# Sovik-Ghosh/SFM

Measured on AMD Instinct MI355X. Metric: BA LM-iterations/sec + descriptor-pairs/sec, 200 cams / 100k pts, 1->8 MI355X, higher is better.
Workload: dtype f64; 1 GPU; BA: 200 cams / 100000 pts / 1000000 obs, cam block 10 (reference 10-parameter block + regulariser), aligned residual order, Huber, SciPy-TRF control flow, fixed schedule; parallelism=points sharded over 1 rank(s), cameras replicated, RCCL all-reduce of [S|r], comm=single rank, seed=1004

## Files before the change

sfm_amd/csrc/ba_model.hip:

```cpp
#include "ba_internal.h"
#include "ba_device.h"

template <int D>
__global__ void k_campre(const double* __restrict__ cams, int C, double fx0, double fy0, double cx0,
                         double cy0, double* __restrict__ out) {
  int c = blockIdx.x * blockDim.x + threadIdx.x;
  if (c >= C) return;
  const double* p = cams + (size_t)c * D;
  const double th2 = p[0] * p[0] + p[1] * p[1] + p[2] * p[2];
  double a, b, a1, b1;
  if (th2 < 1e-4) {
    double z = th2;
    a = 1.0 - z / 6.0 + z * z / 120.0;
    b = 0.5 - z / 24.0 + z * z / 720.0;
    a1 = -1.0 / 3.0 + z / 30.0 - z * z / 840.0;
    b1 = -1.0 / 12.0 + z / 180.0 - z * z / 6720.0;
  } else {
    double t = sqrt(th2), s, co;
    sincos(t, &s, &co);
    a = s / t;
    b = (1.0 - co) / th2;
    a1 = (t * co - s) / (th2 * t);
    b1 = (t * s - 2.0 * (1.0 - co)) / (th2 * th2);
  }
  double* o = out + (size_t)c * CAMPRE;
#pragma unroll
  for (int i = 0; i < 6; ++i) o[i] = p[i];
  if (D == 10) { o[6] = p[6]; o[7] = p[7]; o[8] = p[8]; o[9] = p[9]; }
  else { o[6] = fx0; o[7] = fy0; o[8] = cx0; o[9] = cy0; }
  o[10] = a; o[11] = b; o[12] = a1; o[13] = b1; o[14] = th2; o[15] = 0.0;
}

__device__ __forceinline__ void cam_project(const double* __restrict__ cp, double X0, double X1, double X2,
                                            double& Y0, double& Y1, double& Y2) {
  const double r0 = cp[0], r1 = cp[1], r2 = cp[2], a = cp[10], b = cp[11];
  const double c0 = r1 * X2 - r2 * X1, c1 = r2 * X0 - r0 * X2, c2 = r0 * X1 - r1 * X0;
  const double e0 = r1 * c2 - r2 * c1, e1 = r2 * c0 - r0 * c2, e2 = r0 * c1 - r1 * c0;
  Y0 = X0 + a * c0 + b * e0 + cp[3];
  Y1 = X1 + a * c1 + b * e1 + cp[4];
  Y2 = X2 + a * c2 + b * e2 + cp[5];
}

template <int D, typename T>
__global__ __launch_bounds__(256) void k_lin_obs(int64_t N, const int* __restrict__ cam_idx,
                                                 const int* __restrict__ pt_idx,
                                                 const double* __restrict__ uv,
                                                 const double* __restrict__ pts,
                                                 const double* __restrict__ campre,
                                                 T* __restrict__ recA, T* __restrict__ recB,
                                                 double* __restrict__ part) {
  constexpr int WA = 2 * D, LDA = WA + 1, WB = 8, LDB = WB + 1;
  __shared__ double s_rec[256 * LDA];
  __shared__ double s_red[4];
  const int tid = threadIdx.x;
  const int64_t k0 = (int64_t)blockIdx.x * 256;
  const int64_t k = k0 + tid;
  double cost = 0.0;
  double jb[8];
#pragma unroll
  for (int q = 0; q < 8; ++q) jb[q] = 0.0;
  if (k < N) {
    const int c = cam_idx[k], j = pt_idx[k];
    const double* cp = campre + (size_t)c * CAMPRE;
// ... 41 lines not shown
    const double R10 = a * r2 + b * r1 * r0, R11 = 1.0 + b * (r1 * r1 - th2), R12 = -a * r0 + b * r1 * r2;
    const double R20 = -a * r1 + b * r2 * r0, R21 = a * r0 + b * r2 * r1, R22 = 1.0 + b * (r2 * r2 - th2);
    jb[0] = p00 * R00 + p02 * R20; jb[1] = p00 * R01 + p02 * R21; jb[2] = p00 * R02 + p02 * R22;
    jb[3] = p11 * R10 + p12 * R20; jb[4] = p11 * R11 + p12 * R21; jb[5] = p11 * R12 + p12 * R22;
    jb[6] = ft0; jb[7] = ft1;
  }
  double tot = block_sum256(cost, s_red);
  if (tid == 0) part[blockIdx.x] = tot;
  const int nvalid = (int)((N - k0) < 256 ? (N - k0) : 256);
  {
    T* outp = recA + (size_t)k0 * WA;
    for (int i = tid; i < nvalid * WA; i += 256) {
      const int t = i / WA, q = i - t * WA;
      outp[i] = (T)s_rec[t * LDA + q];
    }
  }
  __syncthreads();
  {
    double* my = &s_rec[tid * LDB];
#pragma unroll
    for (int q = 0; q < 8; ++q) my[q] = jb[q];
  }
  __syncthreads();
  {
    T* outp = recB + (size_t)k0 * WB;
    for (int i = tid; i < nvalid * WB; i += 256) {
      const int t = i >> 3, q = i & 7;
      outp[i] = (T)s_rec[t * LDB + q];
    }
  }
}

template <typename T>
__global__ __launch_bounds__(256) void k_point_blocks(int P, const int* __restrict__ pt_ptr,
                                                      const T* __restrict__ recB,
                                                      double* __restrict__ Cp, double* __restrict__ gp,
                                                      double* __restrict__ part) {
  __shared__ double s_red[4];
  const int j = blockIdx.x * 256 + threadIdx.x;
  double g2 = 0.0, gm = 0.0, cm = 0.0;
  if (j < P) {
    double c0 = 0, c1 = 0, c2 = 0, c3 = 0, c4 = 0, c5 = 0, g0 = 0, g1 = 0, g2v = 0;
    for (int k = pt_ptr[j]; k < pt_ptr[j + 1]; ++k) {
      const T* r = recB + (size_t)k * 8;
      const double a0 = r[0], a1 = r[1], a2 = r[2], b0 = r[3], b1 = r[4], b2 = r[5], f0 = r[6], f1 = r[7];
      c0 += a0 * a0 + b0 * b0; c1 += a0 * a1 + b0 * b1; c2 += a0 * a2 + b0 * b2;
      c3 += a1 * a1 + b1 * b1; c4 += a1 * a2 + b1 * b2; c5 += a2 * a2 + b2 * b2;
      g0 += a0 * f0 + b0 * f1; g1 += a1 * f0 + b1 * f1; g2v += a2 * f0 + b2 * f1;
    }
    double* co = Cp + (size_t)j * 6;
    co[0] = c0; co[1] = c1; co[2] = c2; co[3] = c3; co[4] = c4; co[5] = c5;
    gp[(size_t)j * 3] = g0; gp[(size_t)j * 3 + 1] = g1; gp[(size_t)j * 3 + 2] = g2v;
    g2 = g0 * g0 + g1 * g1 + g2v * g2v;
    gm = fmax(fabs(g0), fmax(fabs(g1), fabs(g2v)));
    cm = fmax(c0, fmax(c3, c5));
  }
  double t2 = block_sum256(g2, s_red);
  double tm = block_max256(gm, s_red);
  double tc = block_max256(cm, s_red);
  if (threadIdx.x == 0) { part[blockIdx.x * 4] = t2; part[blockIdx.x * 4 + 1] = tm; part[blockIdx.x * 4 + 2] = tc; }
}

template <int D, typename T>
__global__ __launch_bounds__(256) void k_cam_blocks_chunks(const int* __restrict__ cch_beg, const int* __restrict__ cch_end,
                                                           const int* __restrict__ cam_obs,
                                                           const T* __restrict__ recA,
                                                           const T* __restrict__ recB, double* __restrict__ part) {
  constexpr int W = 2 * D + 2, LDW = W + 1, NE = D * D + D;
  __shared__ double s[256 * LDW];
  __shared__ double s_tile[4][16 * 17];
  const int ch = blockIdx.x, tid = threadIdx.x, lane = tid & 63, w = tid >> 6;
  const int beg = cch_beg[ch], cnt = cch_end[ch] - beg;
  {
    typedef T pair_t __attribute__((ext_vector_type(2)));
    const int slot = tid >> 4, l16 = tid & 15;
    const bool live = l16 <= D;
    int kk[16];
#pragma unroll
    for (int it = 0; it < 16; ++it) {
      const int o = it * 16 + slot;
      kk[it] = (live && o < cnt) ? cam_obs[beg + o] : -1;
    }
    pair_t v[16];
#pragma unroll
    for (int it = 0; it < 16; ++it) {
      v[it] = (pair_t)(T)0;
      if (kk[it] >= 0)
        v[it] = l16 < D ? *(const pair_t*)(recA + (size_t)kk[it] * (2 * D) + 2 * l16) : *(const pair_t*)(recB + (size_t)kk[it] * 8 + 6);
    }
#pragma unroll
    for (int it = 0; it < 16; ++it) {
      const int o = it * 16 + slot;
      if (kk[it] >= 0) { s[o * LDW + 2 * l16] = (double)v[it].x; s[o * LDW + 2 * l16 + 1] = (double)v[it].y; }
    }
  }
  __syncthreads();
  const int col = lane & 15, kq = lane >> 4;
  const int rrow = kq & 1;
  const int q = col < D ? rrow * D + col : 2 * D + rrow;
  const bool live = col <= D;
  const int per = (cnt + 3) / 4;
  const int wu = __builtin_amdgcn_readfirstlane(w);
  const int o0 = wu * per, o1 = (o0 + per) < cnt ? (o0 + per) : cnt;
  v4d acc = {0.0, 0.0, 0.0, 0.0};
  for (int o = o0; o < o1; o += 8) {
    double v[4];
#pragma unroll
    for (int u = 0; u < 4; ++u) {
      const int oo = o + 2 * u + (kq >> 1);
      v[u] = (live && oo < o1) ? s[oo * LDW + q] : 0.0;
    }
#pragma unroll
    for (int u = 0; u < 4; ++u) {
      if (o + 2 * u >= o1) break;
      acc = __builtin_amdgcn_mfma_f64_16x16x4f64(v[u], v[u], acc, 0, 0, 0);
    }
  }
#pragma unroll
  for (int i = 0; i < 4; ++i) s_tile[w][(kq + 4 * i) * 17 + col] = acc[i];
  __syncthreads();
  if (tid < NE) {
    const int a = tid < D * D ? tid / D : tid - D * D;
    const int b = tid < D * D ? tid - a * D : D;
    part[(size_t)ch * NE + tid] = ((s_tile[0][a * 17 + b] + s_tile[1][a * 17 + b]) + s_tile[2][a * 17 + b]) + s_tile[3][a * 17 + b];
  }
}
template <int D>
__global__ void k_cam_blocks_final(int C, const int* __restrict__ cch_ptr, const double* __restrict__ part,
                                   double* __restrict__ B, double* __restrict__ gc) {
  constexpr int NE = D * D + D;
  const int i = blockIdx.x * blockDim.x + threadIdx.x;
  if (i >= C * NE) return;
  const int c = i / NE, e = i - c * NE;
  double t = 0.0;
  for (int ch = cch_ptr[c]; ch < cch_ptr[c + 1]; ++ch) t += part[(size_t)ch * NE + e];
  if (e < D * D) B[(size_t)c * D * D + e] = t;
  else gc[(size_t)c * D + (e - D * D)] = t;
}

__global__ void k_cam_reg(int C, const double* __restrict__ cams, double fx0, double cx0, double cy0,
                          double width, double height, double w, double* __restrict__ B,
                          double* __restrict__ gc, double* __restrict__ cost_reg,
                          double* __restrict__ regrec) {
  const int c = blockIdx.x * blockDim.x + threadIdx.x;
  if (c >= C) return;
  const double* p = cams + (size_t)c * 10;
  const double fx = p[6], fy = p[7], cx = p[8], cy = p[9];
  double f[4] = {(fx - fx0) / fx0 * w, (fy - fx) / fx * w, (cx - cx0) / width * w, (cy - cy0) / height * w};
  double J[16];
#pragma unroll
  for (int i = 0; i < 16; ++i) J[i] = 0.0;
  J[0] = w / fx0;
  J[4] = -w * fy / (fx * fx); J[5] = w / fx;
  J[10] = w / width;
  J[15] = w / height;
  double cost = 0.0, ft[4];
#pragma unroll
  for (int r = 0; r < 4; ++r) {
    double sc;
    cost += huber_row(f[r], sc, ft[r]);
#pragma unroll
    for (int q = 0; q < 4; ++q) J[r * 4 + q] *= sc;
  }
  cost_reg[c] = 0.5 * cost;
  double* Bc = B + (size_t)c * 100;
#pragma unroll
  for (int i = 0; i < 4; ++i) {
    double g = 0.0;
#pragma unroll
    for (int r = 0; r < 4; ++r) g += J[r * 4 + i] * ft[r];
    gc[(size_t)c * 10 + 6 + i] += g;
#pragma unroll
    for (int q = 0; q < 4; ++q) {
      double hsum = 0.0;
#pragma unroll
      for (int r = 0; r < 4; ++r) hsum += J[r * 4 + i] * J[r * 4 + q];
      Bc[(6 + i) * 10 + 6 + q] += hsum;
    }
  }
  double* rr = regrec + (size_t)c * 20;
#pragma unroll
  for (int i = 0; i < 16; ++i) rr[i] = J[i];
#pragma unroll
  for (int r = 0; r < 4; ++r) rr[16 + r] = ft[r];
}

__global__ __launch_bounds__(256) void k_lin_finalize(int n, int D, const double* __restrict__ gc,
                                                      const double* __restrict__ B,
                                                      const double* __restrict__ part_obs, int nblk_obs,
                                                      const double* __restrict__ part_pt, int nblk_pt,
                                                      const double* __restrict__ cost_reg, int n_reg,
                                                      double* __restrict__ red_lin, double* __restrict__ gmax) {
  __shared__ double s_red[4];
  const int tid = threadIdx.x;
  #pragma unroll 8
  for (int i = tid; i < n; i += 256) {
    red_lin[i] = gc[i];
    const int cam = i / D, a = i - cam * D;
    red_lin[n + 2 + i] = B[(size_t)cam * D * D + a * D + a];
  }
  double c = 0.0, g2 = 0.0, gm = 0.0, cm = 0.0;
  #pragma unroll 8
  for (int i = tid; i < nblk_obs; i += 256) c += part_obs[i];
  #pragma unroll 8
  for (int i = tid; i < n_reg; i += 256) c += cost_reg[i];
  #pragma unroll 8
  for (int i = tid; i < nblk_pt; i += 256) { g2 += part_pt[4 * i]; gm = fmax(gm, part_pt[4 * i + 1]); cm = fmax(cm, part_pt[4 * i + 2]); }
  double ct = block_sum256(c, s_red);
  double g2t = block_sum256(g2, s_red);
  double gmt = block_max256(gm, s_red);
  double cmt = block_max256(cm, s_red);
  if (tid == 0) { red_lin[n] = ct; red_lin[n + 1] = g2t; gmax[0] = gmt; gmax[1] = cmt; }
}

__global__ __launch_bounds__(256) void k_finish_linearize(int n, const double* __restrict__ red_lin,
                                                          const double* __restrict__ gmax,
                                                          double* __restrict__ sc, double* __restrict__ hsc, double seq) {
  __shared__ double s_red[4];
  double g2 = 0.0, gm = 0.0, hm = 0.0;
  #pragma unroll 8
  for (int i = threadIdx.x; i < n; i += 256) {
    double v = red_lin[i]; g2 += v * v; gm = fmax(gm, fabs(v));
    hm = fmax(hm, red_lin[n + 2 + i]);
  }
  double g2t = block_sum256(g2, s_red);
  double gmt = block_max256(gm, s_red);
  double hmt = block_max256(hm, s_red);
  if (threadIdx.x == 0) {
    sc[SFM_SC_COST] = hsc[SFM_SC_COST] = red_lin[n];
    sc[SFM_SC_GNORM2] = hsc[SFM_SC_GNORM2] = g2t + red_lin[n + 1];
    sc[SFM_SC_GINF] = hsc[SFM_SC_GINF] = fmax(gmt, gmax[0]);
    sc[SFM_SC_HDIAG] = hsc[SFM_SC_HDIAG] = fmax(hmt, gmax[1]);
    publish_ticket(hsc, seq);
  }
}

__global__ __launch_bounds__(256) void k_axpy_step(int64_t n_c, int64_t n_total, const double* __restrict__ x,
                                                   const double* __restrict__ pc, const double* __restrict__ pp,
                                                   double scale, double* __restrict__ x_new,
                                                   double* __restrict__ part) {
  __shared__ double s_red[4];
  const int64_t i = (int64_t)blockIdx.x * 256 + threadIdx.x;
  double s2 = 0.0, x2 = 0.0;
  if (i < n_total) {
    const bool is_cam = i < n_c;
    const double s = scale * (is_cam ? pc[i] : pp[i - n_c]);
    const double xn = x[i] + s;
    x_new[i] = xn;
    if (!is_cam) { s2 = s * s; x2 = xn * xn; }
  }
  double a = block_sum256(s2, s_red);
  double b = block_sum256(x2, s_red);
  if (threadIdx.x == 0) { part[blockIdx.x * 2] = a; part[blockIdx.x * 2 + 1] = b; }
}

template <int D, typename T>
__global__ __launch_bounds__(256) void k_step_obs(int64_t N, const int* __restrict__ cam_idx,
                                                  const int* __restrict__ pt_idx,
                                                  const T* __restrict__ recA, const T* __restrict__ recB,
                                                  const double* __restrict__ pc, const double* __restrict__ pp,
                                                  double scale, double* __restrict__ part) {
  __shared__ double s_red[4];
  const int64_t i = (int64_t)blockIdx.x * 256 + threadIdx.x;
  double j2 = 0.0, gt = 0.0;
  if (i < 2 * N) {
    const int64_t k = i >> 1;
    const int row = (int)(i & 1);
    const T* jc = recA + (size_t)k * (2 * D) + row * D;
    const T* rb = recB + (size_t)k * 8;
    const T* jp = rb + row * 3;
    const double* c = pc + (size_t)cam_idx[k] * D;
    const double* q = pp + (size_t)pt_idx[k] * 3;
    double t = (double)jp[0] * q[0] + (double)jp[1] * q[1] + (double)jp[2] * q[2];
#pragma unroll
    for (int a = 0; a < D; ++a) t += (double)jc[a] * c[a];
    t *= scale;
    j2 = t * t;
    gt = (double)rb[6 + row] * t;
  }
  double a = block_sum256(j2, s_red);
  double b = block_sum256(gt, s_red);
  if (threadIdx.x == 0) { part[blockIdx.x * 4] = a; part[blockIdx.x * 4 + 1] = b; }
}

__global__ __launch_bounds__(256) void k_cost_obs(int64_t N, const int* __restrict__ cam_idx,
                                                  const int* __restrict__ pt_idx,
                                                  const double* __restrict__ uv, const double* __restrict__ pts,
                                                  const double* __restrict__ campre,
                                                  double* __restrict__ part, int part_stride, int part_col,
                                                  double* __restrict__ err_out) {
  __shared__ double s_red[4];
  const int64_t k = (int64_t)blockIdx.x * 256 + threadIdx.x;
  double cost = 0.0;
  if (k < N) {
    const double* cp = campre + (size_t)cam_idx[k] * CAMPRE;
    const size_t j = (size_t)pt_idx[k] * 3;
    const double X0 = pts[j], X1 = pts[j + 1], X2 = pts[j + 2];
    double Y0, Y1, Y2;
    cam_project(cp, X0, X1, X2, Y0, Y1, Y2);
    const double iz = 1.0 / Y2;
    const double f0 = cp[6] * (Y0 * iz) + cp[8] - uv[2 * k];
    const double f1 = cp[7] * (Y1 * iz) + cp[9] - uv[2 * k + 1];
    cost = 0.5 * (huber_rho0(f0) + huber_rho0(f1));
    if (err_out) err_out[k] = sqrt(f0 * f0 + f1 * f1);
  }
  double t = block_sum256(cost, s_red);
  if (threadIdx.x == 0 && part) part[(size_t)blockIdx.x * part_stride + part_col] = t;
}

__global__ void k_reg_step(int C, const double* __restrict__ cams_new, const double* __restrict__ pc,
                           double scale, const double* __restrict__ regrec, double fx0, double cx0, double cy0,
                           double width, double height, double w, int with_lin,
                           double* __restrict__ cost_reg ) {
  const int c = blockIdx.x * blockDim.x + threadIdx.x;
  if (c >= C) return;
  const double* p = cams_new + (size_t)c * 10;
  const double fx = p[6], fy = p[7], cx = p[8], cy = p[9];
  const double f[4] = {(fx - fx0) / fx0 * w, (fy - fx) / fx * w, (cx - cx0) / width * w, (cy - cy0) / height * w};
  double cost = 0.0;
#pragma unroll
  for (int r = 0; r < 4; ++r) cost += huber_rho0(f[r]);
  double js2 = 0.0, gts = 0.0;
  if (with_lin) {
    const double* rr = regrec + (size_t)c * 20;
    const double* s = pc + (size_t)c * 10 + 6;
#pragma unroll
    for (int r = 0; r < 4; ++r) {
      const double t = scale * (rr[r * 4] * s[0] + rr[r * 4 + 1] * s[1] + rr[r * 4 + 2] * s[2] + rr[r * 4 + 3] * s[3]);
      js2 += t * t;
      gts += rr[16 + r] * t;
    }
  }
  cost_reg[(size_t)c * 4] = 0.5 * cost;
  cost_reg[(size_t)c * 4 + 1] = js2;
  cost_reg[(size_t)c * 4 + 2] = gts;
}

__global__ __launch_bounds__(256) void k_step_finalize(const double* __restrict__ part_obs, int nblk_obs,
                                                       int nblk_rows, const double* __restrict__ part_x, int nblk_x,
                                                       const double* __restrict__ cost_reg, int n_reg,
                                                       int with_lin, double* __restrict__ red_step) {
  __shared__ double s_red[4];
  double v[5] = {0, 0, 0, 0, 0};
  #pragma unroll 8
  for (int i = threadIdx.x; i < nblk_obs; i += 256) v[2] += part_obs[(size_t)i * 4 + 2];
  if (with_lin)
    #pragma unroll 8
    for (int i = threadIdx.x; i < nblk_rows; i += 256) { v[0] += part_obs[(size_t)i * 4]; v[1] += part_obs[(size_t)i * 4 + 1]; }
  #pragma unroll 8
  for (int i = threadIdx.x; i < n_reg; i += 256) {
    v[2] += cost_reg[(size_t)i * 4]; v[0] += cost_reg[(size_t)i * 4 + 1]; v[1] += cost_reg[(size_t)i * 4 + 2];
  }
  if (with_lin)
    #pragma unroll 8
    for (int i = threadIdx.x; i < nblk_x; i += 256) { v[3] += part_x[(size_t)i * 2]; v[4] += part_x[(size_t)i * 2 + 1]; }
#pragma unroll
  for (int q = 0; q < 5; ++q) {
    double t = block_sum256(v[q], s_red);
    if (threadIdx.x == 0) red_step[q] = t;
  }
}

__global__ __launch_bounds__(256) void k_finish_step(int n_c, const double* __restrict__ pc, double scale,
                                                     const double* __restrict__ x_new,
                                                     const double* __restrict__ red_step,
                                                     double* __restrict__ sc, double* __restrict__ hsc, double seq) {
  __shared__ double s_red[4];
  double s2 = 0.0, x2 = 0.0;
  #pragma unroll 8
  for (int i = threadIdx.x; i < n_c; i += 256) {
    const double s = scale * pc[i];
    s2 += s * s;
    x2 += x_new[i] * x_new[i];
  }
  double a = block_sum256(s2, s_red);
  double b = block_sum256(x2, s_red);
  if (threadIdx.x == 0) {
    sc[SFM_SC_JS2] = hsc[SFM_SC_JS2] = red_step[0]; sc[SFM_SC_GTS] = hsc[SFM_SC_GTS] = red_step[1];
    sc[SFM_SC_COST_NEW] = hsc[SFM_SC_COST_NEW] = red_step[2];
    sc[SFM_SC_SNORM2] = hsc[SFM_SC_SNORM2] = a + red_step[3]; sc[SFM_SC_XNEW_NORM2] = hsc[SFM_SC_XNEW_NORM2] = b + red_step[4];
    publish_ticket(hsc, seq);
  }
}

__global__ void k_set_intrinsics(int C, double fx, double fy, double cx, double cy, double* __restrict__ cp) {
  const int c = blockIdx.x * blockDim.x + threadIdx.x;
  if (c >= C) return;
  double* o = cp + (size_t)c * CAMPRE;
  o[6] = fx; o[7] = fy; o[8] = cx; o[9] = cy;
}

static void launch_projection(sfm_ctx* h, int C, int D, int64_t N, const int* cam_idx, const int* pt_idx, const double* uv,
                              const double* x, double fx, double fy, double cx, double cy, int shared_k, double* campre,
                              double* part, int part_stride, int part_col, double* err_out) {
  DISPATCH_D(D, hipLaunchKernelGGL(k_campre<DD>, dim3(cdiv(C, 64)), dim3(64), 0, h->stream, x, C, fx, fy, cx, cy, campre));
  if (shared_k) hipLaunchKernelGGL(k_set_intrinsics, dim3(cdiv(C, 64)), dim3(64), 0, h->stream, C, fx, fy, cx, cy, campre);
  hipLaunchKernelGGL(k_cost_obs, dim3(cdiv(N, 256)), dim3(256), 0, h->stream, N, cam_idx, pt_idx, uv, x + (size_t)C * D, campre,
                     part, part_stride, part_col, err_out);
}

static int launch_cost(sfm_ctx* h, sfm_ba_problem p, const Lay& L, double* ws, const double* x,
                       const double* pc_for_reg, double scale, int with_lin, double* err_out) {
  const int C = p->n_cams;
  launch_projection(h, p->n_cams, p->cam_dim, p->n_obs, p->cam_idx, p->pt_idx, p->uv, x, p->fx0, p->fy0, p->cx0, p->cy0, 0, WS(L, campre2),
                    WS(L, part_obs), 4, 2, err_out);
  if (p->cam_dim == 10 && p->apply_reg)
    hipLaunchKernelGGL(k_reg_step, dim3(cdiv(C, 64)), dim3(64), 0, h->stream, C, x, pc_for_reg, scale, WS(L, regrec), p->fx0, p->cx0,
                       p->cy0, p->width, p->height, p->reg_weight, with_lin, WS(L, cost_reg));
  SFM_LAUNCH_CHECK(h, "launch_cost");
  return SFM_OK;
}

extern "C" int sfm_ba_cost(sfm_handle h, sfm_ba_problem p, const double* x) {
  Lay L; int rc = check_problem(h, p, &L); if (rc) return rc;
  double* ws = (double*)p->workspace;
  rc = launch_cost(h, p, L, ws, x, nullptr, 0.0, 0, nullptr); if (rc) return rc;
  const int nreg = (p->cam_dim == 10 && p->apply_reg) ? p->n_cams : 0;
  hipLaunchKernelGGL(k_step_finalize, dim3(1), dim3(256), 0, h->stream, WS(L, part_obs), (int)L.nblk_obs, 0,
                     (const double*)nullptr, 0, WS(L, cost_reg), nreg, 0, WS(L, red_step));
  SFM_LAUNCH_CHECK(h, "sfm_ba_cost");
  return SFM_OK;
}

extern "C" int sfm_ba_reproj_errors(sfm_handle h, sfm_ba_problem p, const double* x, int shared_k,
                                    double* err_out) {
  Lay L; int rc = check_problem(h, p, &L); if (rc) return rc;
  if (!err_out) return sfm_fail(h, SFM_ERR_ARG, "sfm_ba_reproj_errors", "null output");
  launch_projection(h, p->n_cams, p->cam_dim, p->n_obs, p->cam_idx, p->pt_idx, p->uv, x, p->fx0, p->fy0, p->cx0, p->cy0, shared_k,
                    (double*)p->workspace + L.campre2, nullptr, 0, 0, err_out);
  SFM_LAUNCH_CHECK(h, "sfm_ba_reproj_errors");
  return SFM_OK;
}

__global__ __launch_bounds__(256) void k_sq_partials(int64_t n, const double* __restrict__ v, double* __restrict__ part) {
  __shared__ double s_red[4];
  const int64_t i = (int64_t)blockIdx.x * 256 + threadIdx.x;
  const double t = i < n ? v[i] * v[i] : 0.0;
  const double a = block_sum256(t, s_red);
  if (threadIdx.x == 0) part[blockIdx.x] = a;
}
extern "C" int sfm_ba_residual_norm2(sfm_handle h, sfm_ba_problem p, const double* x, int shared_k, double* out_host) {
  Lay L; int rc = check_problem(h, p, &L); if (rc) return rc;
  if (!x || !out_host) return sfm_fail(h, SFM_ERR_ARG, "sfm_ba_residual_norm2", "null argument");
  double* ws = (double*)p->workspace;
  launch_projection(h, p->n_cams, p->cam_dim, p->n_obs, p->cam_idx, p->pt_idx, p->uv, x, p->fx0, p->fy0, p->cx0, p->cy0, shared_k, WS(L, campre2),
                    nullptr, 0, 0, WS(L, tmp3));
  hipLaunchKernelGGL(k_sq_partials, dim3((unsigned)L.nblk_obs), dim3(256), 0, h->stream, p->n_obs, WS(L, tmp3), WS(L, part_obs));
  ba_sum_partials(h, WS(L, part_obs), (int)L.nblk_obs, 1, WS(L, red_step) + 6);
  SFM_HIP(h, hipMemcpyAsync(h->pinned + 48, WS(L, red_step) + 6, sizeof(double), hipMemcpyDeviceToHost, h->stream));
  SFM_HIP(h, hipStreamSynchronize(h->stream));
  SFM_LAUNCH_CHECK(h, "sfm_ba_residual_norm2");
  *out_host = h->pinned[48];
  return SFM_OK;
}

extern "C" int sfm_reproj_errors(sfm_handle h, int32_t n_cams, int32_t cam_dim, int64_t n_obs, const int32_t* cam_idx,
                                 const int32_t* pt_idx, const double* uv, const double* x, double fx, double fy, double cx,
                                 double cy, int shared_k, double* err_out) {
  if (!h) return SFM_ERR_ARG;
  if (n_cams < 1 || n_obs < 1 || (cam_dim != 6 && cam_dim != 10) || !cam_idx || !pt_idx || !uv || !x || !err_out)
    return sfm_fail(h, SFM_ERR_ARG, "sfm_reproj_errors", "bad argument");
  double* campre = (double*)sfm_scratch(h, (size_t)n_cams * CAMPRE * sizeof(double));
  if (!campre) return sfm_fail(h, SFM_ERR_HIP, "sfm_reproj_errors", "scratch allocation failed");
  launch_projection(h, n_cams, cam_dim, n_obs, cam_idx, pt_idx, uv, x, fx, fy, cx, cy, shared_k, campre, nullptr, 0, 0, err_out);
  SFM_LAUNCH_CHECK(h, "sfm_reproj_errors");
  return SFM_OK;
}

extern "C" int sfm_ba_linearize(sfm_handle h, sfm_ba_problem p, const double* x) {
  Lay L; int rc = check_problem(h, p, &L); if (rc) return rc;
  double* ws = (double*)p->workspace;
  const int C = p->n_cams, P = p->n_pts, D = p->cam_dim, n = C * D;
  const int64_t N = p->n_obs;
  const double* pts = x + (size_t)n;
  p->cgp.fail_rel *= 0.8;
  DISPATCH_DT(D, p->precision, {
    hipLaunchKernelGGL(k_campre<DD>, dim3(cdiv(C, 64)), dim3(64), 0, h->stream, x, C, p->fx0, p->fy0, p->cx0,
                       p->cy0, WS(L, campre));
    sfm_prof_begin(h, SFM_PROF_LIN_OBS);
    hipLaunchKernelGGL((k_lin_obs<DD, TT>), dim3((unsigned)L.nblk_obs), dim3(256), 0, h->stream, N, p->cam_idx,
                       p->pt_idx, p->uv, pts, WS(L, campre), WST(L, recA), WST(L, recB), WS(L, part_obs));
    sfm_prof_end(h, SFM_PROF_LIN_OBS);
    sfm_prof_begin(h, SFM_PROF_LIN_REST);
    hipLaunchKernelGGL(k_point_blocks<TT>, dim3((unsigned)L.nblk_pt), dim3(256), 0, h->stream, P, p->pt_ptr,
                       WST(L, recB), WS(L, Cp), WS(L, gp), WS(L, part_pt));
    if (p->n_cchunks > 0)
      hipLaunchKernelGGL((k_cam_blocks_chunks<DD, TT>), dim3((unsigned)p->n_cchunks), dim3(256), 0, h->stream, p->cch_beg,
                         p->cch_end, p->cam_obs, WST(L, recA), WST(L, recB), WS(L, cbl_part));
    hipLaunchKernelGGL(k_cam_blocks_final<DD>, dim3(cdiv((int64_t)C * (DD * DD + DD), 256)), dim3(256), 0, h->stream, C,
                       p->cch_ptr, WS(L, cbl_part), WS(L, B), WS(L, gc));
  });
  int nreg = 0;
  if (D == 10 && p->apply_reg) {
    nreg = C;
    hipLaunchKernelGGL(k_cam_reg, dim3(cdiv(C, 64)), dim3(64), 0, h->stream, C, x, p->fx0, p->cx0, p->cy0,
                       p->width, p->height, p->reg_weight, WS(L, B), WS(L, gc), WS(L, cost_reg), WS(L, regrec));
  }
  hipLaunchKernelGGL(k_lin_finalize, dim3(1), dim3(256), 0, h->stream, n, D, WS(L, gc), WS(L, B), WS(L, part_obs),
                     (int)L.nblk_obs, WS(L, part_pt), (int)L.nblk_pt, WS(L, cost_reg), nreg, WS(L, red_lin),
                     WS(L, gmax));
  sfm_prof_end(h, SFM_PROF_LIN_REST);
  SFM_LAUNCH_CHECK(h, "sfm_ba_linearize");
  return SFM_OK;
}

extern "C" int sfm_ba_finish_linearize(sfm_handle h, sfm_ba_problem p) {
  Lay L; int rc = check_problem(h, p, &L); if (rc) return rc;
  double* ws = (double*)p->workspace;
  hipLaunchKernelGGL(k_finish_linearize, dim3(1), dim3(256), 0, h->stream, p->n_cams * p->cam_dim,
                     WS(L, red_lin), WS(L, gmax), WS(L, scalars), p->host_sc, next_ticket(p));
  SFM_LAUNCH_CHECK(h, "sfm_ba_finish_linearize");
  return SFM_OK;
}

extern "C" int sfm_ba_step(sfm_handle h, sfm_ba_problem p, const double* x, double scale, double* x_new) {
  Lay L; int rc = check_problem(h, p, &L); if (rc) return rc;
  double* ws = (double*)p->workspace;
  const int C = p->n_cams, P = p->n_pts, D = p->cam_dim, n = C * D;
  const int64_t N = p->n_obs, ntot = (int64_t)n + 3 * (int64_t)P;
  double* part_x = WS(L, part_x);
  sfm_prof_begin(h, SFM_PROF_STEP);
  const unsigned nblk_x = cdiv(ntot, 256), nblk_rows = cdiv(2 * N, 256);
  hipLaunchKernelGGL(k_axpy_step, dim3(nblk_x), dim3(256), 0, h->stream, (int64_t)n, ntot, x, WS(L, pc), WS(L, pp),
                     scale, x_new, part_x);
  DISPATCH_DT(D, p->precision, hipLaunchKernelGGL((k_step_obs<DD, TT>), dim3(nblk_rows), dim3(256), 0, h->stream, N, p->cam_idx,
                                                  p->pt_idx, WST(L, recA), WST(L, recB), WS(L, pc), WS(L, pp), scale, WS(L, part_obs)));
  rc = launch_cost(h, p, L, ws, x_new, WS(L, pc), scale, 1, nullptr); if (rc) return rc;
  const int nreg = (D == 10 && p->apply_reg) ? C : 0;
  hipLaunchKernelGGL(k_step_finalize, dim3(1), dim3(256), 0, h->stream, WS(L, part_obs), (int)L.nblk_obs,
                     (int)nblk_rows, part_x, (int)nblk_x, WS(L, cost_reg), nreg, 1, WS(L, red_step));
  sfm_prof_end(h, SFM_PROF_STEP);
  SFM_LAUNCH_CHECK(h, "sfm_ba_step");
  return SFM_OK;
}

extern "C" int sfm_ba_finish_step(sfm_handle h, sfm_ba_problem p, const double* x, double scale,
                                  const double* x_new) {
  Lay L; int rc = check_problem(h, p, &L); if (rc) return rc;
  double* ws = (double*)p->workspace;
  (void)x;
  hipLaunchKernelGGL(k_finish_step, dim3(1), dim3(256), 0, h->stream, p->n_cams * p->cam_dim, WS(L, pc), scale,
                     x_new, WS(L, red_step), WS(L, scalars), p->host_sc, next_ticket(p));
  SFM_LAUNCH_CHECK(h, "sfm_ba_finish_step");
  return SFM_OK;
}

__global__ __launch_bounds__(256) void k_xnorm_finish(int n_c, const double* __restrict__ x, const double* __restrict__ red_step,
                                                      double* __restrict__ sc, double* __restrict__ hsc, double seq) {
  __shared__ double s_red[4];
  double a = 0.0;
  for (int i = threadIdx.x; i < n_c; i += 256) a += x[i] * x[i];
  const double t = block_sum256(a, s_red);
  if (threadIdx.x == 0) { sc[SFM_SC_XNEW_NORM2] = hsc[SFM_SC_XNEW_NORM2] = t + red_step[4]; publish_ticket(hsc, seq); }
}
int ba_xnorm_partial(sfm_ctx* h, sfm_ba_problem p, const double* x) {
  Lay L; int rc = check_problem(h, p, &L); if (rc) return rc;
  double* ws = (double*)p->workspace;
  const int64_t n = (int64_t)p->n_cams * p->cam_dim, np3 = 3 * (int64_t)p->n_pts;
  const unsigned nb = cdiv(np3, 256);
  hipLaunchKernelGGL(k_sq_partials, dim3(nb), dim3(256), 0, h->stream, np3, x + n, WS(L, part_x));
  ba_sum_partials(h, WS(L, part_x), (int)nb, 1, WS(L, red_step) + 4);
  SFM_LAUNCH_CHECK(h, "ba_xnorm_partial");
// ... 10 lines not shown
```

Before: 250.4 LM-iterations/s.

## Fuse BA linearize and step kernels to cut launches and serial reductions

Point-block and camera-chunk Hessian kernels are merged into one launch, and the camera regulariser is folded into a per-camera final reduction kernel. The step path fuses the axpy with camera precompute and regulariser evaluation, and merges the step-obs and cost kernels into one pass. The single-block finalize reductions are spread over several blocks. The aim is to remove kernel launch overhead and serial single-block reductions, at the price of more complex kernels with branch-divergent block roles and higher register or LDS pressure.

After: 253.2 LM-iterations/s (median of 6 runs). +1.1%, better.

```diff
diff --git a/sfm_amd/csrc/ba_model.hip b/sfm_amd/csrc/ba_model.hip
--- a/sfm_amd/csrc/ba_model.hip
+++ b/sfm_amd/csrc/ba_model.hip
@@ -2,11 +2,7 @@
 #include "ba_device.h"
 
 template <int D>
-__global__ void k_campre(const double* __restrict__ cams, int C, double fx0, double fy0, double cx0,
-                         double cy0, double* __restrict__ out) {
-  int c = blockIdx.x * blockDim.x + threadIdx.x;
-  if (c >= C) return;
-  const double* p = cams + (size_t)c * D;
+__device__ __forceinline__ void campre_row(const double (&p)[D], double fx0, double fy0, double cx0, double cy0, double* __restrict__ o) {
   const double th2 = p[0] * p[0] + p[1] * p[1] + p[2] * p[2];
   double a, b, a1, b1;
   if (th2 < 1e-4) {
@@ -23,12 +19,21 @@
     a1 = (t * co - s) / (th2 * t);
     b1 = (t * s - 2.0 * (1.0 - co)) / (th2 * th2);
   }
-  double* o = out + (size_t)c * CAMPRE;
 #pragma unroll
   for (int i = 0; i < 6; ++i) o[i] = p[i];
   if (D == 10) { o[6] = p[6]; o[7] = p[7]; o[8] = p[8]; o[9] = p[9]; }
   else { o[6] = fx0; o[7] = fy0; o[8] = cx0; o[9] = cy0; }
   o[10] = a; o[11] = b; o[12] = a1; o[13] = b1; o[14] = th2; o[15] = 0.0;
+}
+template <int D>
+__global__ void k_campre(const double* __restrict__ cams, int C, double fx0, double fy0, double cx0,
+                         double cy0, double* __restrict__ out) {
+  int c = blockIdx.x * blockDim.x + threadIdx.x;
+  if (c >= C) return;
+  double p[D];
+#pragma unroll
+  for (int i = 0; i < D; ++i) p[i] = cams[(size_t)c * D + i];
+  campre_row<D>(p, fx0, fy0, cx0, cy0, out + (size_t)c * CAMPRE);
 }
 
 __device__ __forceinline__ void cam_project(const double* __restrict__ cp, double X0, double X1, double X2,
@@ -136,12 +141,12 @@
 }
 
 template <typename T>
-__global__ __launch_bounds__(256) void k_point_blocks(int P, const int* __restrict__ pt_ptr,
-                                                      const T* __restrict__ recB,
-                                                      double* __restrict__ Cp, double* __restrict__ gp,
-                                                      double* __restrict__ part) {
-  __shared__ double s_red[4];
-  const int j = blockIdx.x * 256 + threadIdx.x;
+__device__ __forceinline__ void point_blocks_wg(int blk, int P, const int* __restrict__ pt_ptr,
+                                                const T* __restrict__ recB,
+                                                double* __restrict__ Cp, double* __restrict__ gp,
+                                                double* __restrict__ part) {
+  __shared__ double s_red[4];
+  const int j = blk * 256 + threadIdx.x;
   double g2 = 0.0, gm = 0.0, cm = 0.0;
   if (j < P) {
     double c0 = 0, c1 = 0, c2 = 0, c3 = 0, c4 = 0, c5 = 0, g0 = 0, g1 = 0, g2v = 0;
@@ -162,18 +167,18 @@
   double t2 = block_sum256(g2, s_red);
   double tm = block_max256(gm, s_red);
   double tc = block_max256(cm, s_red);
-  if (threadIdx.x == 0) { part[blockIdx.x * 4] = t2; part[blockIdx.x * 4 + 1] = tm; part[blockIdx.x * 4 + 2] = tc; }
+  if (threadIdx.x == 0) { part[blk * 4] = t2; part[blk * 4 + 1] = tm; part[blk * 4 + 2] = tc; }
 }
 
 template <int D, typename T>
-__global__ __launch_bounds__(256) void k_cam_blocks_chunks(const int* __restrict__ cch_beg, const int* __restrict__ cch_end,
-                                                           const int* __restrict__ cam_obs,
-                                                           const T* __restrict__ recA,
-                                                           const T* __restrict__ recB, double* __restrict__ part) {
+__device__ __forceinline__ void cam_blocks_chunk_wg(int ch, const int* __restrict__ cch_beg, const int* __restrict__ cch_end,
+                                                    const int* __restrict__ cam_obs,
+                                                    const T* __restrict__ recA,
+                                                    const T* __restrict__ recB, double* __restrict__ part) {
   constexpr int W = 2 * D + 2, LDW = W + 1, NE = D * D + D;
   __shared__ double s[256 * LDW];
   __shared__ double s_tile[4][16 * 17];
-  const int ch = blockIdx.x, tid = threadIdx.x, lane = tid & 63, w = tid >> 6;
+  const int tid = threadIdx.x, lane = tid & 63, w = tid >> 6;
   const int beg = cch_beg[ch], cnt = cch_end[ch] - beg;
   {
     typedef T pair_t __attribute__((ext_vector_type(2)));
@@ -229,26 +234,19 @@
     part[(size_t)ch * NE + tid] = ((s_tile[0][a * 17 + b] + s_tile[1][a * 17 + b]) + s_tile[2][a * 17 + b]) + s_tile[3][a * 17 + b];
   }
 }
-template <int D>
-__global__ void k_cam_blocks_final(int C, const int* __restrict__ cch_ptr, const double* __restrict__ part,
-                                   double* __restrict__ B, double* __restrict__ gc) {
-  constexpr int NE = D * D + D;
-  const int i = blockIdx.x * blockDim.x + threadIdx.x;
-  if (i >= C * NE) return;
-  const int c = i / NE, e = i - c * NE;
-  double t = 0.0;
-  for (int ch = cch_ptr[c]; ch < cch_ptr[c + 1]; ++ch) t += part[(size_t)ch * NE + e];
-  if (e < D * D) B[(size_t)c * D * D + e] = t;
-  else gc[(size_t)c * D + (e - D * D)] = t;
-}
-
-__global__ void k_cam_reg(int C, const double* __restrict__ cams, double fx0, double cx0, double cy0,
-                          double width, double height, double w, double* __restrict__ B,
-                          double* __restrict__ gc, double* __restrict__ cost_reg,
-                          double* __restrict__ regrec) {
-  const int c = blockIdx.x * blockDim.x + threadIdx.x;
-  if (c >= C) return;
-  const double* p = cams + (size_t)c * 10;
+template <int D, typename T>
+__global__ __launch_bounds__(256) void k_point_cam_blocks(int P, const int* __restrict__ pt_ptr, const T* __restrict__ recB,
+                                                          double* __restrict__ Cp, double* __restrict__ gp,
+                                                          double* __restrict__ part_pt, unsigned nblk_pt,
+                                                          const int* __restrict__ cch_beg, const int* __restrict__ cch_end,
+                                                          const int* __restrict__ cam_obs, const T* __restrict__ recA,
+                                                          double* __restrict__ cbl_part) {
+  if (blockIdx.x < nblk_pt) point_blocks_wg<T>((int)blockIdx.x, P, pt_ptr, recB, Cp, gp, part_pt);
+  else cam_blocks_chunk_wg<D, T>((int)(blockIdx.x - nblk_pt), cch_beg, cch_end, cam_obs, recA, recB, cbl_part);
+}
+__device__ __forceinline__ void cam_reg_rows(const double* __restrict__ p, double fx0, double cx0, double cy0,
+                                             double width, double height, double w, double* Bc, double* gcc,
+                                             double* __restrict__ cost_reg, double* __restrict__ rr) {
   const double fx = p[6], fy = p[7], cx = p[8], cy = p[9];
   double f[4] = {(fx - fx0) / fx0 * w, (fy - fx) / fx * w, (cx - cx0) / width * w, (cy - cy0) / height * w};
   double J[16];
@@ -266,14 +264,13 @@
 #pragma unroll
     for (int q = 0; q < 4; ++q) J[r * 4 + q] *= sc;
   }
-  cost_reg[c] = 0.5 * cost;
-  double* Bc = B + (size_t)c * 100;
+  *cost_reg = 0.5 * cost;
 #pragma unroll
   for (int i = 0; i < 4; ++i) {
     double g = 0.0;
 #pragma unroll
     for (int r = 0; r < 4; ++r) g += J[r * 4 + i] * ft[r];
-    gc[(size_t)c * 10 + 6 + i] += g;
+    gcc[6 + i] += g;
 #pragma unroll
     for (int q = 0; q < 4; ++q) {
       double hsum = 0.0;
@@ -282,13 +279,41 @@
       Bc[(6 + i) * 10 + 6 + q] += hsum;
     }
   }
-  double* rr = regrec + (size_t)c * 20;
 #pragma unroll
   for (int i = 0; i < 16; ++i) rr[i] = J[i];
 #pragma unroll
   for (int r = 0; r < 4; ++r) rr[16 + r] = ft[r];
 }
 
+template <int D>
+__global__ __launch_bounds__(128) void k_cam_blocks_final(const int* __restrict__ cch_ptr, const double* __restrict__ part,
+                                                          double* __restrict__ B, double* __restrict__ gc, int with_reg,
+                                                          const double* __restrict__ cams, double fx0, double cx0, double cy0,
+                                                          double width, double height, double w,
+                                                          double* __restrict__ cost_reg, double* __restrict__ regrec) {
+  constexpr int NE = D * D + D;
+  static_assert(NE <= 128, "one thread per element of [B_c | g_c]");
+  __shared__ double s_v[NE];
+  const int c = blockIdx.x, e = threadIdx.x;
+  if (e < NE) {
+    double t = 0.0;
+    const int ch1 = cch_ptr[c + 1];
+#pragma unroll 8
+    for (int ch = cch_ptr[c]; ch < ch1; ++ch) t += part[(size_t)ch * NE + e];
+    s_v[e] = t;
+  }
+  if constexpr (D == 10) {
+    if (with_reg) {
+      __syncthreads();
+      if (e == 0) cam_reg_rows(cams + (size_t)c * 10, fx0, cx0, cy0, width, height, w, s_v, s_v + 100, cost_reg + c, regrec + (size_t)c * 20);
+    }
+  }
+  __syncthreads();
+  if (e < D * D) B[(size_t)c * D * D + e] = s_v[e];
+  else if (e < NE) gc[(size_t)c * D + (e - D * D)] = s_v[e];
+}
+
+constexpr int LIN_FINALIZE_COLS = 4;
 __global__ __launch_bounds__(256) void k_lin_finalize(int n, int D, const double* __restrict__ gc,
                                                       const double* __restrict__ B,
                                                       const double* __restrict__ part_obs, int nblk_obs,
@@ -296,25 +321,37 @@
                                                       const double* __restrict__ cost_reg, int n_reg,
                                                       double* __restrict__ red_lin, double* __restrict__ gmax) {
   __shared__ double s_red[4];
-  const int tid = threadIdx.x;
-  #pragma unroll 8
-  for (int i = tid; i < n; i += 256) {
-    red_lin[i] = gc[i];
-    const int cam = i / D, a = i - cam * D;
-    red_lin[n + 2 + i] = B[(size_t)cam * D * D + a * D + a];
-  }
-  double c = 0.0, g2 = 0.0, gm = 0.0, cm = 0.0;
-  #pragma unroll 8
-  for (int i = tid; i < nblk_obs; i += 256) c += part_obs[i];
-  #pragma unroll 8
-  for (int i = tid; i < n_reg; i += 256) c += cost_reg[i];
-  #pragma unroll 8
-  for (int i = tid; i < nblk_pt; i += 256) { g2 += part_pt[4 * i]; gm = fmax(gm, part_pt[4 * i + 1]); cm = fmax(cm, part_pt[4 * i + 2]); }
-  double ct = block_sum256(c, s_red);
-  double g2t = block_sum256(g2, s_red);
-  double gmt = block_max256(gm, s_red);
-  double cmt = block_max256(cm, s_red);
-  if (tid == 0) { red_lin[n] = ct; red_lin[n + 1] = g2t; gmax[0] = gmt; gmax[1] = cmt; }
+  const int tid = threadIdx.x, col = blockIdx.x;
+  if (col >= LIN_FINALIZE_COLS) {
+    const int i = (col - LIN_FINALIZE_COLS) * 256 + tid;
+    if (i < n) {
+      red_lin[i] = gc[i];
+      const int cam = i / D, a = i - cam * D;
+      red_lin[n + 2 + i] = B[(size_t)cam * D * D + a * D + a];
+    }
+    return;
+  }
+  if (col == 0) {
+    double c = 0.0;
+    #pragma unroll 8
+    for (int i = tid; i < nblk_obs; i += 256) c += part_obs[i];
+    #pragma unroll 8
+    for (int i = tid; i < n_reg; i += 256) c += cost_reg[i];
+    const double ct = block_sum256(c, s_red);
+    if (tid == 0) red_lin[n] = ct;
+  } else if (col == 1) {
+    double g2 = 0.0;
+    #pragma unroll 8
+    for (int i = tid; i < nblk_pt; i += 256) g2 += part_pt[4 * i];
+    const double g2t = block_sum256(g2, s_red);
+    if (tid == 0) red_lin[n + 1] = g2t;
+  } else {
+    double m = 0.0;
+    #pragma unroll 8
+    for (int i = tid; i < nblk_pt; i += 256) m = fmax(m, part_pt[4 * i + col - 1]);
+    const double mt = block_max256(m, s_red);
+    if (tid == 0) gmax[col - 2] = mt;
+  }
 }
 
 __global__ __launch_bounds__(256) void k_finish_linearize(int n, const double* __restrict__ red_lin,
@@ -339,17 +376,67 @@
   }
 }
 
+__device__ __forceinline__ void reg_step_rows(const double* p , const double* __restrict__ s ,
+                                              double scale, const double* __restrict__ rr, double fx0, double cx0, double cy0,
+                                              double width, double height, double w, int with_lin,
+                                              double* __restrict__ out ) {
+  const double fx = p[6], fy = p[7], cx = p[8], cy = p[9];
+  const double f[4] = {(fx - fx0) / fx0 * w, (fy - fx) / fx * w, (cx - cx0) / width * w, (cy - cy0) / height * w};
+  double cost = 0.0;
+#pragma unroll
+  for (int r = 0; r < 4; ++r) cost += huber_rho0(f[r]);
+  double js2 = 0.0, gts = 0.0;
+  if (with_lin) {
+#pragma unroll
+    for (int r = 0; r < 4; ++r) {
+      const double t = scale * (rr[r * 4] * s[0] + rr[r * 4 + 1] * s[1] + rr[r * 4 + 2] * s[2] + rr[r * 4 + 3] * s[3]);
+      js2 += t * t;
+      gts += rr[16 + r] * t;
+    }
+  }
+  out[0] = 0.5 * cost;
+  out[1] = js2;
+  out[2] = gts;
+}
+__global__ void k_reg_step(int C, const double* __restrict__ cams_new, const double* __restrict__ pc,
+                           double scale, const double* __restrict__ regrec, double fx0, double cx0, double cy0,
+                           double width, double height, double w, int with_lin,
+                           double* __restrict__ cost_reg ) {
+  const int c = blockIdx.x * blockDim.x + threadIdx.x;
+  if (c >= C) return;
+  reg_step_rows(cams_new + (size_t)c * 10, pc + (size_t)c * 10 + 6, scale, regrec + (size_t)c * 20, fx0, cx0, cy0, width, height, w,
+                with_lin, cost_reg + (size_t)c * 4);
+}
+
+__device__ __forceinline__ double axpy_val(double x, double scale, double p) { return fma(scale, p, x); }
+template <int D>
 __global__ __launch_bounds__(256) void k_axpy_step(int64_t n_c, int64_t n_total, const double* __restrict__ x,
                                                    const double* __restrict__ pc, const double* __restrict__ pp,
                                                    double scale, double* __restrict__ x_new,
-                                                   double* __restrict__ part) {
+                                                   double* __restrict__ part, unsigned nblk_x, int C, double fx0, double fy0,
+                                                   double cx0, double cy0, double* __restrict__ campre2,
+                                                   const double* __restrict__ regrec, double width, double height, double w,
+                                                   double* __restrict__ cost_reg) {
+  if (blockIdx.x >= nblk_x) {
+    const unsigned nblk_c = (unsigned)(C + 255) / 256, b = blockIdx.x - nblk_x;
+    const int c = (int)(b < nblk_c ? b : b - nblk_c) * 256 + (int)threadIdx.x;
+    if (c >= C) return;
+    double p[D];
+#pragma unroll
+    for (int i = 0; i < D; ++i) p[i] = axpy_val(x[(size_t)c * D + i], scale, pc[(size_t)c * D + i]);
+    if (b < nblk_c) campre_row<D>(p, fx0, fy0, cx0, cy0, campre2 + (size_t)c * CAMPRE);
+    else if constexpr (D == 10)
+      reg_step_rows(p, pc + (size_t)c * 10 + 6, scale, regrec + (size_t)c * 20, fx0, cx0, cy0, width, height, w, 1, cost_reg + (size_t)c * 4);
+    return;
+  }
   __shared__ double s_red[4];
   const int64_t i = (int64_t)blockIdx.x * 256 + threadIdx.x;
   double s2 = 0.0, x2 = 0.0;
   if (i < n_total) {
     const bool is_cam = i < n_c;
-    const double s = scale * (is_cam ? pc[i] : pp[i - n_c]);
-    const double xn = x[i] + s;
+    const double pv = is_cam ? pc[i] : pp[i - n_c];
+    const double s = scale * pv;
+    const double xn = axpy_val(x[i], scale, pv);
     x_new[i] = xn;
     if (!is_cam) { s2 = s * s; x2 = xn * xn; }
   }
@@ -359,32 +446,100 @@
 }
 
 template <int D, typename T>
-__global__ __launch_bounds__(256) void k_step_obs(int64_t N, const int* __restrict__ cam_idx,
-                                                  const int* __restrict__ pt_idx,
-                                                  const T* __restrict__ recA, const T* __restrict__ recB,
-                                                  const double* __restrict__ pc, const double* __restrict__ pp,
-                                                  double scale, double* __restrict__ part) {
-  __shared__ double s_red[4];
-  const int64_t i = (int64_t)blockIdx.x * 256 + threadIdx.x;
-  double j2 = 0.0, gt = 0.0;
-  if (i < 2 * N) {
-    const int64_t k = i >> 1;
-    const int row = (int)(i & 1);
-    const T* jc = recA + (size_t)k * (2 * D) + row * D;
-    const T* rb = recB + (size_t)k * 8;
-    const T* jp = rb + row * 3;
-    const double* c = pc + (size_t)cam_idx[k] * D;
-    const double* q = pp + (size_t)pt_idx[k] * 3;
-    double t = (double)jp[0] * q[0] + (double)jp[1] * q[1] + (double)jp[2] * q[2];
-#pragma unroll
-    for (int a = 0; a < D; ++a) t += (double)jc[a] * c[a];
-    t *= scale;
-    j2 = t * t;
-    gt = (double)rb[6 + row] * t;
-  }
-  double a = block_sum256(j2, s_red);
-  double b = block_sum256(gt, s_red);
-  if (threadIdx.x == 0) { part[blockIdx.x * 4] = a; part[blockIdx.x * 4 + 1] = b; }
+__global__ __launch_bounds__(256) void k_step_cost_obs(int64_t N, const int* __restrict__ cam_idx,
+                                                       const int* __restrict__ pt_idx, const double* __restrict__ uv,
+                                                       const T* __restrict__ recA, const T* __restrict__ recB,
+                                                       const double* __restrict__ pc, const double* __restrict__ pp,
+                                                       double scale, const double* __restrict__ pts_new,
+                                                       const double* __restrict__ campre2, double* __restrict__ part) {
+  constexpr int WA = 2 * D, LDA = WA + 1, LDB = 9;
+  constexpr int VE = 16 / (int)sizeof(T);
+  constexpr int NA = WA / VE, NB = 8 / VE;
+  static_assert(WA % VE == 0 && 8 % VE == 0, "record rows are whole 16-byte pieces");
+  __shared__ double s_buf[256 * LDA];
+  __shared__ double s_j2[512], s_gt[512];
+  __shared__ double s_red[5][4];
+  typedef T vec_t __attribute__((ext_vector_type(VE)));
+  const int tid = threadIdx.x;
+  const int64_t k0 = (int64_t)blockIdx.x * 256;
+  const int nvalid = (int)((N - k0) < 256 ? (N - k0) : 256);
+  const bool live = tid < nvalid;
+  const int64_t k = k0 + tid;
+  const size_t cam = live ? cam_idx[k] : 0, pj = live ? pt_idx[k] : 0;
+  vec_t la[NA], lb[NB];
+  {
+    const vec_t* inA = (const vec_t*)(recA + (size_t)k0 * WA);
+    const vec_t* inB = (const vec_t*)(recB + (size_t)k0 * 8);
+#pragma unroll
+    for (int j = 0; j < NB; ++j) { const int i = tid + 256 * j; lb[j] = i * VE < nvalid * 8 ? inB[i] : (vec_t)(T)0; }
+#pragma unroll
+    for (int j = 0; j < NA; ++j) { const int i = tid + 256 * j; la[j] = i * VE < nvalid * WA ? inA[i] : (vec_t)(T)0; }
+  }
+  const double u0 = live ? uv[2 * k] : 0.0, u1 = live ? uv[2 * k + 1] : 0.0;
+  double c[D], q[3], cp[CAMPRE - 1], X[3];
+#pragma unroll
+  for (int a = 0; a < D; ++a) c[a] = pc[cam * D + a];
+#pragma unroll
+  for (int a = 0; a < 3; ++a) q[a] = pp[pj * 3 + a];
+#pragma unroll
+  for (int a = 0; a < CAMPRE - 1; ++a) cp[a] = campre2[cam * CAMPRE + a];
+#pragma unroll
+  for (int a = 0; a < 3; ++a) X[a] = pts_new[pj * 3 + a];
+#pragma unroll
+  for (int j = 0; j < NB; ++j)
+#pragma unroll
+    for (int v = 0; v < VE; ++v) { const int i = (tid + 256 * j) * VE + v; s_buf[(i >> 3) * LDB + (i & 7)] = (double)lb[j][v]; }
+  __syncthreads();
+  double jb[8];
+#pragma unroll
+  for (int e = 0; e < 8; ++e) jb[e] = s_buf[tid * LDB + e];
+  __syncthreads();
+#pragma unroll
+  for (int j = 0; j < NA; ++j)
+#pragma unroll
+    for (int v = 0; v < VE; ++v) { const int i = (tid + 256 * j) * VE + v, t = i / WA, e = i - t * WA; s_buf[t * LDA + e] = (double)la[j][v]; }
+  __syncthreads();
+  double cost = 0.0;
+#pragma unroll
+  for (int row = 0; row < 2; ++row) {
+    double t = 0.0, fr = 0.0;
+    if (live) {
+      const double* jc = &s_buf[tid * LDA + row * D];
+      const double* jp = &jb[row * 3];
+      t = jp[0] * q[0] + jp[1] * q[1] + jp[2] * q[2];
+#pragma unroll
+      for (int a = 0; a < D; ++a) t += jc[a] * c[a];
+      t *= scale;
+      fr = jb[6 + row];
+    }
+    s_j2[2 * tid + row] = t * t;
+    s_gt[2 * tid + row] = fr * t;
+  }
+  if (live) {
+    double Y0, Y1, Y2;
+    cam_project(cp, X[0], X[1], X[2], Y0, Y1, Y2);
+    const double iz = 1.0 / Y2;
+    const double f0 = cp[6] * (Y0 * iz) + cp[8] - u0;
+    const double f1 = cp[7] * (Y1 * iz) + cp[9] - u1;
+    cost = 0.5 * (huber_rho0(f0) + huber_rho0(f1));
+  }
+  __syncthreads();
+  double w[5] = {s_j2[tid], s_gt[tid], cost, s_j2[256 + tid], s_gt[256 + tid]};
+#pragma unroll
+  for (int e = 0; e < 5; ++e) w[e] = wave_sum(w[e]);
+  if ((tid & 63) == 0)
+#pragma unroll
+    for (int e = 0; e < 5; ++e) s_red[e][tid >> 6] = w[e];
+  __syncthreads();
+  if (tid == 0) {
+    double tot[5];
+#pragma unroll
+    for (int e = 0; e < 5; ++e) tot[e] = s_red[e][0] + s_red[e][1] + s_red[e][2] + s_red[e][3];
+    const size_t b = blockIdx.x;
+    part[8 * b] = tot[0]; part[8 * b + 1] = tot[1];
+    part[4 * b + 2] = tot[2];
+    if (nvalid > 128) { part[8 * b + 4] = tot[3]; part[8 * b + 5] = tot[4]; }
+  }
 }
 
 __global__ __launch_bounds__(256) void k_cost_obs(int64_t N, const int* __restrict__ cam_idx,
@@ -412,57 +567,30 @@
   if (threadIdx.x == 0 && part) part[(size_t)blockIdx.x * part_stride + part_col] = t;
 }
 
-__global__ void k_reg_step(int C, const double* __restrict__ cams_new, const double* __restrict__ pc,
-                           double scale, const double* __restrict__ regrec, double fx0, double cx0, double cy0,
-                           double width, double height, double w, int with_lin,
-                           double* __restrict__ cost_reg ) {
-  const int c = blockIdx.x * blockDim.x + threadIdx.x;
-  if (c >= C) return;
-  const double* p = cams_new + (size_t)c * 10;
-  const double fx = p[6], fy = p[7], cx = p[8], cy = p[9];
-  const double f[4] = {(fx - fx0) / fx0 * w, (fy - fx) / fx * w, (cx - cx0) / width * w, (cy - cy0) / height * w};
-  double cost = 0.0;
-#pragma unroll
-  for (int r = 0; r < 4; ++r) cost += huber_rho0(f[r]);
-  double js2 = 0.0, gts = 0.0;
-  if (with_lin) {
-    const double* rr = regrec + (size_t)c * 20;
-    const double* s = pc + (size_t)c * 10 + 6;
-#pragma unroll
-    for (int r = 0; r < 4; ++r) {
-      const double t = scale * (rr[r * 4] * s[0] + rr[r * 4 + 1] * s[1] + rr[r * 4 + 2] * s[2] + rr[r * 4 + 3] * s[3]);
-      js2 += t * t;
-      gts += rr[16 + r] * t;
-    }
-  }
-  cost_reg[(size_t)c * 4] = 0.5 * cost;
-  cost_reg[(size_t)c * 4 + 1] = js2;
-  cost_reg[(size_t)c * 4 + 2] = gts;
-}
-
 __global__ __launch_bounds__(256) void k_step_finalize(const double* __restrict__ part_obs, int nblk_obs,
                                                        int nblk_rows, const double* __restrict__ part_x, int nblk_x,
                                                        const double* __restrict__ cost_reg, int n_reg,
                                                        int with_lin, double* __restrict__ red_step) {
   __shared__ double s_red[4];
-  double v[5] = {0, 0, 0, 0, 0};
-  #pragma unroll 8
-  for (int i = threadIdx.x; i < nblk_obs; i += 256) v[2] += part_obs[(size_t)i * 4 + 2];
-  if (with_lin)
+  const int q = blockIdx.x;
+  double v = 0.0;
+  if (q == 2) {
     #pragma unroll 8
-    for (int i = threadIdx.x; i < nblk_rows; i += 256) { v[0] += part_obs[(size_t)i * 4]; v[1] += part_obs[(size_t)i * 4 + 1]; }
-  #pragma unroll 8
-  for (int i = threadIdx.x; i < n_reg; i += 256) {
-    v[2] += cost_reg[(size_t)i * 4]; v[0] += cost_reg[(size_t)i * 4 + 1]; v[1] += cost_reg[(size_t)i * 4 + 2];
-  }
-  if (with_lin)
+    for (int i = threadIdx.x; i < nblk_obs; i += 256) v += part_obs[(size_t)i * 4 + 2];
     #pragma unroll 8
-    for (int i = threadIdx.x; i < nblk_x; i += 256) { v[3] += part_x[(size_t)i * 2]; v[4] += part_x[(size_t)i * 2 + 1]; }
-#pragma unroll
-  for (int q = 0; q < 5; ++q) {
-    double t = block_sum256(v[q], s_red);
-    if (threadIdx.x == 0) red_step[q] = t;
-  }
+    for (int i = threadIdx.x; i < n_reg; i += 256) v += cost_reg[(size_t)i * 4];
+  } else if (q < 2) {
+    if (with_lin)
+      #pragma unroll 8
+      for (int i = threadIdx.x; i < nblk_rows; i += 256) v += part_obs[(size_t)i * 4 + q];
+    #pragma unroll 8
+    for (int i = threadIdx.x; i < n_reg; i += 256) v += cost_reg[(size_t)i * 4 + 1 + q];
+  } else if (with_lin) {
+    #pragma unroll 8
+    for (int i = threadIdx.x; i < nblk_x; i += 256) v += part_x[(size_t)i * 2 + (q - 3)];
+  }
+  const double t = block_sum256(v, s_red);
+  if (threadIdx.x == 0) red_step[q] = t;
 }
 
 __global__ __launch_bounds__(256) void k_finish_step(int n_c, const double* __restrict__ pc, double scale,
@@ -520,7 +648,7 @@
   double* ws = (double*)p->workspace;
   rc = launch_cost(h, p, L, ws, x, nullptr, 0.0, 0, nullptr); if (rc) return rc;
   const int nreg = (p->cam_dim == 10 && p->apply_reg) ? p->n_cams : 0;
-  hipLaunchKernelGGL(k_step_finalize, dim3(1), dim3(256), 0, h->stream, WS(L, part_obs), (int)L.nblk_obs, 0,
+  hipLaunchKernelGGL(k_step_finalize, dim3(5), dim3(256), 0, h->stream, WS(L, part_obs), (int)L.nblk_obs, 0,
                      (const double*)nullptr, 0, WS(L, cost_reg), nreg, 0, WS(L, red_step));
   SFM_LAUNCH_CHECK(h, "sfm_ba_cost");
   return SFM_OK;
@@ -577,6 +705,7 @@
   const int C = p->n_cams, P = p->n_pts, D = p->cam_dim, n = C * D;
   const int64_t N = p->n_obs;
   const double* pts = x + (size_t)n;
+  const int nreg = (D == 10 && p->apply_reg) ? C : 0;
   p->cgp.fail_rel *= 0.8;
   DISPATCH_DT(D, p->precision, {
     hipLaunchKernelGGL(k_campre<DD>, dim3(cdiv(C, 64)), dim3(64), 0, h->stream, x, C, p->fx0, p->fy0, p->cx0,
@@ -586,28 +715,19 @@
                        p->pt_idx, p->uv, pts, WS(L, campre), WST(L, recA), WST(L, recB), WS(L, part_obs));
     sfm_prof_end(h, SFM_PROF_LIN_OBS);
     sfm_prof_begin(h, SFM_PROF_LIN_REST);
-    hipLaunchKernelGGL(k_point_blocks<TT>, dim3((unsigned)L.nblk_pt), dim3(256), 0, h->stream, P, p->pt_ptr,
-                       WST(L, recB), WS(L, Cp), WS(L, gp), WS(L, part_pt));
-    if (p->n_cchunks > 0)
-      hipLaunchKernelGGL((k_cam_blocks_chunks<DD, TT>), dim3((unsigned)p->n_cchunks), dim3(256), 0, h->stream, p->cch_beg,
-                         p->cch_end, p->cam_obs, WST(L, recA), WST(L, recB), WS(L, cbl_part));
-    hipLaunchKernelGGL(k_cam_blocks_final<DD>, dim3(cdiv((int64_t)C * (DD * DD + DD), 256)), dim3(256), 0, h->stream, C,
-                       p->cch_ptr, WS(L, cbl_part), WS(L, B), WS(L, gc));
+    hipLaunchKernelGGL((k_point_cam_blocks<DD, TT>), dim3((unsigned)L.nblk_pt + (unsigned)p->n_cchunks), dim3(256), 0, h->stream, P,
+                       p->pt_ptr, WST(L, recB), WS(L, Cp), WS(L, gp), WS(L, part_pt), (unsigned)L.nblk_pt, p->cch_beg, p->cch_end,
+                       p->cam_obs, WST(L, recA), WS(L, cbl_part));
+    hipLaunchKernelGGL(k_cam_blocks_final<DD>, dim3(C), dim3(128), 0, h->stream, p->cch_ptr, WS(L, cbl_part), WS(L, B), WS(L, gc),
+                       nreg > 0, x, p->fx0, p->cx0, p->cy0, p->width, p->height, p->reg_weight, WS(L, cost_reg), WS(L, regrec));
   });
-  int nreg = 0;
-  if (D == 10 && p->apply_reg) {
-    nreg = C;
-    hipLaunchKernelGGL(k_cam_reg, dim3(cdiv(C, 64)), dim3(64), 0, h->stream, C, x, p->fx0, p->cx0, p->cy0,
-                       p->width, p->height, p->reg_weight, WS(L, B), WS(L, gc), WS(L, cost_reg), WS(L, regrec));
-  }
-  hipLaunchKernelGGL(k_lin_finalize, dim3(1), dim3(256), 0, h->stream, n, D, WS(L, gc), WS(L, B), WS(L, part_obs),
+  hipLaunchKernelGGL(k_lin_finalize, dim3(LIN_FINALIZE_COLS + cdiv(n, 256)), dim3(256), 0, h->stream, n, D, WS(L, gc), WS(L, B), WS(L, part_obs),
                      (int)L.nblk_obs, WS(L, part_pt), (int)L.nblk_pt, WS(L, cost_reg), nreg, WS(L, red_lin),
                      WS(L, gmax));
   sfm_prof_end(h, SFM_PROF_LIN_REST);
   SFM_LAUNCH_CHECK(h, "sfm_ba_linearize");
   return SFM_OK;
 }
-
 extern "C" int sfm_ba_finish_linearize(sfm_handle h, sfm_ba_problem p) {
   Lay L; int rc = check_problem(h, p, &L); if (rc) return rc;
   double* ws = (double*)p->workspace;
@@ -625,13 +745,14 @@
   double* part_x = WS(L, part_x);
   sfm_prof_begin(h, SFM_PROF_STEP);
   const unsigned nblk_x = cdiv(ntot, 256), nblk_rows = cdiv(2 * N, 256);
-  hipLaunchKernelGGL(k_axpy_step, dim3(nblk_x), dim3(256), 0, h->stream, (int64_t)n, ntot, x, WS(L, pc), WS(L, pp),
-                     scale, x_new, part_x);
-  DISPATCH_DT(D, p->precision, hipLaunchKernelGGL((k_step_obs<DD, TT>), dim3(nblk_rows), dim3(256), 0, h->stream, N, p->cam_idx,
-                                                  p->pt_idx, WST(L, recA), WST(L, recB), WS(L, pc), WS(L, pp), scale, WS(L, part_obs)));
-  rc = launch_cost(h, p, L, ws, x_new, WS(L, pc), scale, 1, nullptr); if (rc) return rc;
   const int nreg = (D == 10 && p->apply_reg) ? C : 0;
-  hipLaunchKernelGGL(k_step_finalize, dim3(1), dim3(256), 0, h->stream, WS(L, part_obs), (int)L.nblk_obs,
+  DISPATCH_D(D, hipLaunchKernelGGL(k_axpy_step<DD>, dim3(nblk_x + cdiv(C, 256) * (nreg > 0 ? 2 : 1)), dim3(256), 0, h->stream, (int64_t)n, ntot, x, WS(L, pc),
+                                   WS(L, pp), scale, x_new, part_x, nblk_x, C, p->fx0, p->fy0, p->cx0, p->cy0, WS(L, campre2),
+                                   WS(L, regrec), p->width, p->height, p->reg_weight, WS(L, cost_reg)));
+  DISPATCH_DT(D, p->precision, hipLaunchKernelGGL((k_step_cost_obs<DD, TT>), dim3((unsigned)L.nblk_obs), dim3(256), 0, h->stream, N,
+                                                  p->cam_idx, p->pt_idx, p->uv, WST(L, recA), WST(L, recB), WS(L, pc), WS(L, pp), scale,
+                                                  x_new + (size_t)n, WS(L, campre2), WS(L, part_obs)));
+  hipLaunchKernelGGL(k_step_finalize, dim3(5), dim3(256), 0, h->stream, WS(L, part_obs), (int)L.nblk_obs,
                      (int)nblk_rows, part_x, (int)nblk_x, WS(L, cost_reg), nreg, 1, WS(L, red_step));
   sfm_prof_end(h, SFM_PROF_STEP);
   SFM_LAUNCH_CHECK(h, "sfm_ba_step");
```
